# ZhaoyangLyu/Point_Diffusion_Refinement

Measured on AMD Instinct MI355X. Metric: DDPM reverse steps/sec (T=1000, N=2048), higher is better.
Workload: dtype f32; 1 GPU; BASELINE configs[1]: B=32/GPU, N=2048, 3072-pt mirrored condition, T=1000 DDPM reverse sampling, random-init dual-path PointNet++ (9.76 M params), cached condition step; global_batch=32, parallelism=dp1, launch=hipGraph replay, noise=device Philox, execution=fused channel-last HIP

## Files before the change

### point_diffusion_refinement_amd/csrc/fused_layer_ws.hip

```cpp
#include <cstdlib>

#include "layer_tiles.h"

#include <type_traits>

namespace {

typedef float f32x16 __attribute__((ext_vector_type(16)));
typedef float f32x2 __attribute__((ext_vector_type(2)));
typedef float f32x4 __attribute__((ext_vector_type(4)));

#ifdef PDR_LAB_TRACE
__device__ unsigned long long pdr_lab_trace[3][4096];
__device__ unsigned long long pdr_lab_wg[2048][3];
#define PDR_T(role, slot)                                                                   \
  do {                                                                                      \
    if (trace_on && (threadIdx.x & 63) == 0 && (slot) < 4096)                               \
      pdr_lab_trace[role][slot] = __builtin_amdgcn_s_memtime();                             \
  } while (0)
#else
#define PDR_T(role, slot) do {} while (0)
#endif

constexpr int kMaxCin = 4096;
__device__ float k_ones[kMaxCin + 8] = {[0 ... kMaxCin + 7] = 1.0f};
__device__ float k_zeros[kMaxCin + 8] = {[0 ... kMaxCin + 7] = 0.0f};

__device__ __forceinline__ float vmax(float a, float b) {
  float r;
  asm("v_max_f32 %0, %1, %2" : "=v"(r) : "v"(a), "v"(b));
  return r;
}

template <bool SPLIT, int KC, int TM, int TN>
struct StageMem;
template <int KC, int TM, int TN>
struct StageMem<false, KC, TM, TN> {
  static constexpr int APAD = KC == 32 ? 1 : 2;
  __attribute__((aligned(8))) float As[2][KC / 2][TM + APAD][2];
  __attribute__((aligned(16))) float Bs[2][KC][TN];
};
template <int KC, int TM, int TN>
struct StageMem<true, KC, TM, TN> {
  static_assert(KC == 32, "split layout: 32 halves = 64-byte rows");
  __attribute__((aligned(16))) unsigned char A[2][2][TM * 64];
  __attribute__((aligned(16))) unsigned char B[2][2][TN * 64];
};

typedef _Float16 half8 __attribute__((ext_vector_type(8)));
typedef _Float16 half2v __attribute__((ext_vector_type(2)));

__device__ __forceinline__ int split_off(int r, int g) { return r * 64 + ((g ^ ((r >> 2) & 3)) << 4); }

template <int RT, int CT, bool RADD, bool SPLIT>
constexpr int ws_waves_per_simd() { return (RT * CT == 1 && !RADD && !SPLIT) ? 6 : 4; }

template <int RT, int CT, int WR, int WC, int KC, bool RADD, int GATH = 0, bool SPLIT = false, bool POOL = false,
          bool PAIR = false>
__global__ __launch_bounds__(512, (ws_waves_per_simd<RT, CT, RADD, SPLIT>())) void fused_layer_ws_kernel(
    pdr_layer_in_t in_a, int Cin, const float* __restrict__ Wt, int ldw,
    const float* __restrict__ bias, int Cout, float* __restrict__ Y_a, int ldy_a,
    float* __restrict__ partial_a, int relu_col0, int n_row_tiles_a, int tile_order, pdr::PoolArgs pool,
    pdr::WsTwin tw) {
  static_assert(!PAIR || (!RADD && !SPLIT && !POOL && GATH != 2), "paired launches: plain / ball-gathered, no residual");
  const int sel = PAIR ? __builtin_amdgcn_readfirstlane(static_cast<int>(blockIdx.x) >= tw.gx ? 1 : 0) : 0;
  const bool second = PAIR && sel != 0;
  const pdr_layer_in_t& in = PAIR ? tw.in[sel] : in_a;
  float* const __restrict__ Y = PAIR ? tw.Y[sel] : Y_a;
  float* const __restrict__ partial = PAIR ? tw.partial[sel] : partial_a;
  const int ldy = PAIR ? tw.ldy[sel] : ldy_a;
  const int n_row_tiles = PAIR ? tw.n_row_tiles[sel] : n_row_tiles_a;
  const int vbx = (PAIR && second) ? static_cast<int>(blockIdx.x) - tw.gx : static_cast<int>(blockIdx.x);
  const int vnwg = PAIR ? (second ? static_cast<int>(gridDim.x) - tw.gx : tw.gx) : static_cast<int>(gridDim.x);
  static_assert(WR * WC == 4, "4 consumer waves");
  constexpr int TM = WR * RT * 32, TN = WC * CT * 32;
  static_assert(!SPLIT || TN == 128 || TN == 64, "split image: 128- or 64-column blocks");
  constexpr int C4 = KC / 4;
  constexpr int PT = 256;
  constexpr int VSTEP = PT / C4;
  constexpr int APT4 = TM / VSTEP;
  constexpr int TN4 = TN / 4;
  constexpr int WPT4 = (KC * TN4 + PT - 1) / PT;
  static_assert(TM % VSTEP == 0, "tile rows");
  __shared__ StageMem<SPLIT, KC, TM, TN> sm;
  __shared__ float red[WR][TN][2];
  __shared__ int epi_ticket;
  __shared__ __attribute__((aligned(16))) float Tt[4][16][36];

  const int tid = threadIdx.x;
  const int wave = __builtin_amdgcn_readfirstlane(tid >> 6);
  const int rpb = in.rows_per_batch;
  const int tpb = (rpb + TM - 1) / TM;
  const int n0 = blockIdx.y * TN;
  int nch = 0;
  for (int s = 0; s < in.n_seg; ++s) nch += (in.seg[s].C + KC - 1) / KC;
  const int nwg = vnwg;
  const int nB = n_row_tiles / tpb;
  const bool listed = in.tile_list != nullptr;
  const bool xcd_order = !listed && tile_order != 0 && (nwg & 7) == 0 && nB >= 8 && (nB & 7) == 0;
  const int xcd = vbx & 7;
  const int tile_first = xcd_order ? vbx >> 3 : vbx;
  const int tile_step = xcd_order ? nwg >> 3 : nwg;
  const int tile_limit = listed ? min(*in.n_tiles, n_row_tiles)
                                : (xcd_order ? ((nB - xcd + 7) >> 3) * tpb : n_row_tiles);
  const bool rev = in.walk_reverse != 0 && !listed;
  auto row_tile = [&](int l) __attribute__((always_inline)) -> int {
    return listed ? in.tile_list[l] : (rev ? tile_limit - 1 - l : l);
  };
  const int ptpb = in.partial_tpb > 0 ? in.partial_tpb : tpb;
  const int cloud_mul = xcd_order ? 8 : 1, cloud_add = xcd_order ? xcd : 0;
  const int my_tiles = tile_limit > tile_first ? (tile_limit - tile_first + tile_step - 1) / tile_step : 0;
  if constexpr (POOL) {
    if (in.patch_values) {
      constexpr int TN4p = TN / 4;
      constexpr int QP = 512 / TN4p;
      const int Kp = pool.K;
      const long nq = static_cast<long>(n_row_tiles) * TM / Kp;
      const int qpb = rpb / Kp;
      const int c = n0 + 4 * (tid % TN4p);
      const float lo = pool.v_relu ? 0.0f : -__builtin_inff();
      if (tid < QP * TN4p && c < Cout) {
        for (long q = static_cast<long>(blockIdx.x) * QP + tid / TN4p; q < nq; q += static_cast<long>(gridDim.x) * QP) {
          if (in.patch_w[q] > 0.0f) {
            const long bq = q / qpb;
            const f32x4 v = *reinterpret_cast<const f32x4*>(in.patch_values + q * in.patch_ld + c);
            f32x4 sc = {1.0f, 1.0f, 1.0f, 1.0f}, sh = {0.0f, 0.0f, 0.0f, 0.0f};
            if (pool.vscale) sc = *reinterpret_cast<const f32x4*>(pool.vscale + bq * Cout + c);
            if (pool.vshift) sh = *reinterpret_cast<const f32x4*>(pool.vshift + bq * Cout + c);
            f32x4 o;
#pragma unroll
            for (int j = 0; j < 4; ++j) o[j] = vmax(__builtin_fmaf(v[j], sc[j], sh[j]), lo);
            const long orow = in.out_rows ? static_cast<long>(in.out_rows[q]) : q;
            *reinterpret_cast<f32x4*>(pool.out + orow * pool.ldo + c) = o;
          }
        }
      }
    }
  }
  if (my_tiles == 0) return;
#ifdef PDR_LAB_TRACE
  if (tid == 0 && blockIdx.y == 0 && blockIdx.x < 2048) {
    unsigned xcc;
    asm volatile("s_getreg_b32 %0, hwreg(HW_REG_XCC_ID)" : "=s"(xcc));
    pdr_lab_wg[blockIdx.x][0] = __builtin_amdgcn_s_memrealtime();
    pdr_lab_wg[blockIdx.x][2] = (xcc & 15) | (static_cast<unsigned long long>(my_tiles) << 8);
  }
#endif
  const int G = my_tiles * nch;
  const bool has_partial = partial != nullptr;
  if (tid == 0) epi_ticket = 0;
#ifdef PDR_LAB_TRACE
  const bool trace_on = blockIdx.x == 37 % gridDim.x && blockIdx.y == 0 && (wave == 0 || wave == 4 || wave == 6);
#endif

  struct Cur { int tile, sg, ks, cbase, ci; };
  auto advance = [&](Cur& c, bool really = true) {
    const int segC = in.seg[c.sg].C;
    const int ks1 = c.ks + KC;
    const bool seg_end = ks1 >= segC;
    const bool tile_end = seg_end && (c.sg + 1 >= in.n_seg);
    Cur n;
    n.ks = seg_end ? 0 : ks1;
    n.cbase = tile_end ? 0 : (seg_end ? c.cbase + segC : c.cbase);
    n.sg = tile_end ? 0 : (seg_end ? c.sg + 1 : c.sg);
    n.tile = tile_end ? c.tile + tile_step : c.tile;
    n.ci = tile_end ? 0 : c.ci + 1;
    c.ci = really ? n.ci : c.ci;
    c.ks = really ? n.ks : c.ks;
    c.cbase = really ? n.cbase : c.cbase;
    c.sg = really ? n.sg : c.sg;
    c.tile = really ? n.tile : c.tile;
  };
  auto last_of_tile = [&](const Cur& c) { return c.sg == in.n_seg - 1 && c.ks + KC >= in.seg[c.sg].C; };

  if (wave >= 4) {
#ifndef PDR_LAB_NO_PRIO
    __builtin_amdgcn_s_setprio(3);
#endif
    if constexpr (SPLIT) {
      __builtin_amdgcn_s_setreg(1 | (23 << 6) | (0 << 11), 1);
    }
    const float lo_pre = in.pre_relu ? 0.0f : -__builtin_inff();
    const float lo_post = in.post_relu ? 0.0f : -__builtin_inff();
    const int pt = tid - 256;
    const int vc4 = pt % C4, vr0 = pt / C4;
    constexpr bool ROWQ = GATH != 0;
    const int gsh_ = (GATH && in.gK > 0) ? __builtin_ctz(in.gK) : 0;
    auto prow = [&](int i) __attribute__((always_inline)) -> int { return ROWQ ? APT4 * vr0 + i : vr0 + VSTEP * i; };
    const int ss_ld = in.ss_ld > 0 ? in.ss_ld : Cin;
    const bool has_pre = in.pre_relu != 0, has_add = in.add != nullptr;
    unsigned a_off[APT4], r_off[RADD ? APT4 : 1], w_off[WPT4];
    int off_sg = -1;
    {
      const int nmax = ldw - n0 - 4;
#pragma unroll
      for (int i = 0; i < WPT4; ++i) {
        const int e = pt + PT * i;
        const int k = e / TN4, n4 = e - k * TN4;
        w_off[i] = static_cast<unsigned>(min(k, KC - 1) * ldw + min(4 * n4, nmax)) * 4u;
      }
      if constexpr (RADD) {
#pragma unroll
        for (int i = 0; i < APT4; ++i)
          r_off[i] = static_cast<unsigned>(prow(i) * in.rseg.ld + 4 * vc4) * 4u;
      }
    }
    int g_idx[GATH ? APT4 : 1], n_idx[GATH == 1 ? APT4 : 1], n_cnt = 1;
    unsigned v_off = 0;
    auto load_idx = [&](long r0, int nv, int (&id)[GATH ? APT4 : 1], int& cnt) __attribute__((always_inline)) {
      if constexpr (GATH != 0) {
        const int rf = min(APT4 * vr0, nv - 1);
        cnt = in.gcnt ? in.gcnt[(r0 + rf) >> gsh_] : 1;
        if (nv == TM) {
          __builtin_memcpy(&id[0], in.gidx + r0 + APT4 * vr0, sizeof(int) * APT4);
        } else {
#pragma unroll
          for (int i = 0; i < APT4; ++i) id[i] = in.gidx[r0 + min(APT4 * vr0 + i, nv - 1)];
        }
      }
    };
    constexpr bool KNN = GATH == 2;
    float gs1v[KNN ? APT4 : 1], gs2v[KNN ? APT4 : 1];
    f32x4 Rq1, Rq2;
    int g_tile = -1, n_tile = -1;
    const int gsh = (GATH && in.gK > 0) ? __builtin_ctz(in.gK) : 0;
    bool Rgath = false;
    constexpr bool RG = RADD && GATH != 0;
    float4 Rrv[APT4], Rrv2[1];
    f32x4 Rrrv[RADD ? APT4 : 1], Rrrv2[1], Rqr1, Rqr2;
    f32x4 Rrw[WPT4];
    float Rps[4], Rph[4], Rpa[4];
    int Rkmax = KC, Rcvalid = 4;
    auto fetch = [&](const Cur& c) __attribute__((always_inline)) {
      const int lt = row_tile(c.tile);
      const int bl = lt / tpb, tb = lt - bl * tpb;
      const int b = bl * cloud_mul + cloud_add;
#ifdef PDR_LAB_SAME_ROWS
      const long row0 = static_cast<long>(tb & 1) * TM;
#else
      const long row0 = static_cast<long>(b) * rpb + static_cast<long>(tb) * TM;
#endif
      const int nvalid = min(TM, rpb - tb * TM);
      const pdr_seg_t seg = in.seg[c.sg];
      const int shift = __builtin_ctz(seg.row_div);
      Rkmax = min(KC, seg.C - c.ks);
      const float* sc_b = (in.scale ? in.scale + static_cast<long>(b) * ss_ld : k_ones) + c.cbase + c.ks;
      const float* sh_b = (in.shift ? in.shift + static_cast<long>(b) * ss_ld : k_zeros) + c.cbase + c.ks;
      const float* ad_b = (in.add ? in.add + static_cast<long>(b) * in.add_ld : k_zeros) + c.cbase + c.ks;
      const bool f_g = GATH && seg.gV != nullptr;
      if constexpr (GATH) {
        if (c.tile != g_tile && (!PAIR || in.gidx)) {
          off_sg = -1;
          if (GATH == 1 && c.tile == n_tile) {
#pragma unroll
            for (int i = 0; i < APT4; ++i) g_idx[i] = n_cnt <= 0 ? -1 : n_idx[i];
          } else {
            int cnt = 1;
            load_idx(row0, nvalid, g_idx, cnt);
#pragma unroll
            for (int i = 0; i < APT4; ++i) g_idx[i] = cnt <= 0 ? -1 : g_idx[i];
          }
          if constexpr (KNN) {
            if (nvalid == TM) {
              __builtin_memcpy(&gs1v[0], in.gs1 + row0 + APT4 * vr0, sizeof(float) * APT4);
              __builtin_memcpy(&gs2v[0], in.gs2 + row0 + APT4 * vr0, sizeof(float) * APT4);
            } else {
#pragma unroll
              for (int i = 0; i < APT4; ++i) {
                const long p = row0 + min(prow(i), nvalid - 1);
                gs1v[i] = in.gs1[p];
                gs2v[i] = in.gs2[p];
              }
            }
          }
          g_tile = c.tile;
        }
        const int nt = c.tile + tile_step;
        if (GATH == 1 && last_of_tile(c) && nt < tile_limit && (!PAIR || in.gidx)) {
          const int nlt = row_tile(nt);
          const int nbl = nlt / tpb, ntb = nlt - nbl * tpb;
          const int nb = nbl * cloud_mul + cloud_add;
          const long nrow0 = static_cast<long>(nb) * rpb + static_cast<long>(ntb) * TM;
          const int nnv = min(TM, rpb - ntb * TM);
          if constexpr (GATH == 1) load_idx(nrow0, nnv, n_idx, n_cnt);
          n_tile = nt;
        }
      }
      const char* ab = reinterpret_cast<const char*>(
          seg.ptr + (f_g ? static_cast<long>(b) * seg.g_nsrc : (row0 >> shift)) * seg.ld + c.ks);
      const int zrow = f_g ? seg.g_zrow - b * seg.g_nsrc : 0;
      const int v0d = (f_g && seg.gV0) ? static_cast<int>(seg.gV0 - seg.gV) : 0;
      const char* wb = SPLIT ? reinterpret_cast<const char*>(Wt) +
                                   (static_cast<long>(blockIdx.y) * ldw + c.ci) * (2L * TN * 64)
                             : reinterpret_cast<const char*>(Wt + static_cast<long>(c.cbase + c.ks) * ldw + n0);
      unsigned ao[APT4], ro[RADD ? APT4 : 1], wo[WPT4], po[4], vo = 0;
      if (Rkmax == KC && nvalid == TM) {
        if (off_sg != c.sg) {
          off_sg = c.sg;
#pragma unroll
          for (int i = 0; i < APT4; ++i) {
            int row = prow(i) >> shift;
            if constexpr (GATH) {
              if (f_g) {
                row = g_idx[i] < 0 ? zrow : g_idx[i];
                if (i == 0)
                  v_off = static_cast<unsigned>((prow(0) >> gsh) * seg.g_ldv + 4 * vc4 + (g_idx[0] < 0 ? v0d : 0)) * 4u;
              }
            }
            a_off[i] = static_cast<unsigned>(row * seg.ld + 4 * vc4) * 4u;
          }
        }
        if constexpr (GATH) vo = v_off;
        Rcvalid = 4;
#pragma unroll
        for (int j = 0; j < 4; ++j) po[j] = 16u * vc4 + 4u * j;
#pragma unroll
        for (int i = 0; i < APT4; ++i) ao[i] = a_off[i];
        if constexpr (RADD) {
#pragma unroll
          for (int i = 0; i < APT4; ++i) ro[i] = r_off[i];
        }
#pragma unroll
        for (int i = 0; i < WPT4; ++i) wo[i] = SPLIT ? static_cast<unsigned>(pt + PT * i) * 16u : w_off[i];
      } else {
        const int cl = 4 * vc4;
        const int clc = min(cl, ((seg.C + 3) & ~3) - 4 - c.ks);
        Rcvalid = cl == clc ? min(4, seg.C - c.ks - clc) : 0;
#pragma unroll
        for (int j = 0; j < 4; ++j) po[j] = static_cast<unsigned>(min(clc + j, seg.C - 1 - c.ks)) * 4u;
#pragma unroll
        for (int i = 0; i < APT4; ++i) {
          const int r = min(prow(i), nvalid - 1);
          int row = r >> shift;
          if constexpr (GATH) {
            if (f_g) {
              row = g_idx[i] < 0 ? zrow : g_idx[i];
              if (i == 0) vo = static_cast<unsigned>((r >> gsh) * seg.g_ldv + clc + (g_idx[0] < 0 ? v0d : 0)) * 4u;
            }
          }
          ao[i] = static_cast<unsigned>(row * seg.ld + clc) * 4u;
          if constexpr (RADD) ro[i] = static_cast<unsigned>(r * in.rseg.ld + clc) * 4u;
        }
        const int nmax = ldw - n0 - 4;
#pragma unroll
        for (int i = 0; i < WPT4; ++i) {
          const int e = pt + PT * i;
          const int k = e / TN4, n4 = e - k * TN4;
          wo[i] = SPLIT ? static_cast<unsigned>(pt + PT * i) * 16u
                        : static_cast<unsigned>(min(k, Rkmax - 1) * ldw + min(4 * n4, nmax)) * 4u;
        }
      }
      if (Rkmax == KC) {
        f32x4 s4, h4, a4;
        __builtin_memcpy(&s4, reinterpret_cast<const char*>(sc_b) + 16u * vc4, 16);
        __builtin_memcpy(&h4, reinterpret_cast<const char*>(sh_b) + 16u * vc4, 16);
        __builtin_memcpy(&a4, reinterpret_cast<const char*>(ad_b) + 16u * vc4, 16);
#pragma unroll
        for (int j = 0; j < 4; ++j) {
          Rps[j] = s4[j];
          Rph[j] = h4[j];
          Rpa[j] = a4[j];
        }
      } else {
#pragma unroll
        for (int j = 0; j < 4; ++j) {
          Rps[j] = *reinterpret_cast<const float*>(reinterpret_cast<const char*>(sc_b) + po[j]);
          Rph[j] = *reinterpret_cast<const float*>(reinterpret_cast<const char*>(sh_b) + po[j]);
          Rpa[j] = *reinterpret_cast<const float*>(reinterpret_cast<const char*>(ad_b) + po[j]);
        }
      }
#pragma unroll
      for (int i = 0; i < APT4; ++i) Rrv[i] = *reinterpret_cast<const float4*>(ab + ao[i]);
      if constexpr (GATH) {
        Rgath = f_g;
        if (f_g) {
          const char* vb = reinterpret_cast<const char*>(seg.gV + (row0 >> gsh) * seg.g_ldv + c.ks);
          Rrv2[0] = *reinterpret_cast<const float4*>(vb + vo);
          if constexpr (KNN) {
            const unsigned qo = Rkmax == KC ? 16u * vc4
                                            : static_cast<unsigned>(min(4 * vc4, ((seg.C + 3) & ~3) - 4 - c.ks)) * 4u;
            __builtin_memcpy(&Rq1, reinterpret_cast<const char*>(seg.g_r1 + c.ks) + qo, 16);
            __builtin_memcpy(&Rq2, reinterpret_cast<const char*>(seg.g_r2 + c.ks) + qo, 16);
          }
        }
      }
      if constexpr (RG) {
        const int rs_ld = in.rseg.ld, rs_ldv = in.rseg.g_ldv, rs_nsrc = in.rseg.g_nsrc;
        const char* rb = reinterpret_cast<const char*>(in.rseg.ptr + static_cast<long>(b) * rs_nsrc * rs_ld +
                                                       c.cbase + c.ks);
        const char* rvb = reinterpret_cast<const char*>(in.rseg.gV + (row0 >> gsh) * rs_ldv + c.cbase + c.ks);
        const int rz = in.rseg.g_zrow - b * rs_nsrc;
        const int rv0d = in.rseg.gV0 ? static_cast<int>(in.rseg.gV0 - in.rseg.gV) : 0;
        const bool fast = Rkmax == KC && nvalid == TM;
        const int colq = fast ? 4 * vc4 : min(4 * vc4, ((Cin + 3) & ~3) - 4 - c.cbase - c.ks);
#pragma unroll
        for (int i = 0; i < APT4; ++i) {
          const int urow = g_idx[i] < 0 ? rz : g_idx[i];
          Rrrv[i] = *reinterpret_cast<const f32x4*>(rb + static_cast<unsigned>(urow * rs_ld + colq) * 4u);
        }
        Rrrv2[0] = *reinterpret_cast<const f32x4*>(
            rvb + static_cast<unsigned>((min(prow(0), nvalid - 1) >> gsh) * rs_ldv + colq +
                                        (g_idx[0] < 0 ? rv0d : 0)) * 4u);
        if constexpr (GATH == 2) {
          __builtin_memcpy(&Rqr1, in.rseg.g_r1 + c.cbase + c.ks + colq, 16);
          __builtin_memcpy(&Rqr2, in.rseg.g_r2 + c.cbase + c.ks + colq, 16);
        }
      } else if constexpr (RADD) {
        const char* rb = reinterpret_cast<const char*>(in.rseg.ptr + row0 * in.rseg.ld + c.cbase + c.ks);
#pragma unroll
        for (int i = 0; i < APT4; ++i) Rrrv[i] = *reinterpret_cast<const f32x4*>(rb + ro[i]);
      }
#pragma unroll
      for (int i = 0; i < WPT4; ++i) Rrw[i] = *reinterpret_cast<const f32x4*>(wb + wo[i]);
    };
    auto commit = [&](int st) __attribute__((always_inline)) {
      auto stage_a = [&](auto masked, auto pre, auto add) __attribute__((always_inline)) {
        constexpr bool MASKED = decltype(masked)::value, PRE = decltype(pre)::value, ADD = decltype(add)::value;
#pragma unroll
        for (int i = 0; i < APT4; ++i) {
          float x[4] = {Rrv[i].x, Rrv[i].y, Rrv[i].z, Rrv[i].w};
          if constexpr (GATH) {
            if (Rgath) {
              x[0] += Rrv2[0].x; x[1] += Rrv2[0].y; x[2] += Rrv2[0].z; x[3] += Rrv2[0].w;
              if constexpr (KNN) {
#pragma unroll
                for (int j = 0; j < 4; ++j) {
                  x[j] = __builtin_fmaf(gs1v[i], Rq1[j], x[j]);
                  x[j] = __builtin_fmaf(gs2v[i], Rq2[j], x[j]);
                }
              }
            }
          }
          float q[4] = {0.0f, 0.0f, 0.0f, 0.0f};
          if constexpr (RADD) {
            q[0] = Rrrv[i][0]; q[1] = Rrrv[i][1]; q[2] = Rrrv[i][2]; q[3] = Rrrv[i][3];
            if constexpr (RG) {
              q[0] += Rrrv2[0][0]; q[1] += Rrrv2[0][1]; q[2] += Rrrv2[0][2]; q[3] += Rrrv2[0][3];
              if constexpr (GATH == 2) {
#pragma unroll
                for (int j = 0; j < 4; ++j) {
                  q[j] = __builtin_fmaf(gs1v[i], Rqr1[j], q[j]);
                  q[j] = __builtin_fmaf(gs2v[i], Rqr2[j], q[j]);
                }
              }
            }
          }
#pragma unroll
          for (int j = 0; j < 4; ++j) {
            float v = x[j];
            if constexpr (PRE) v = vmax(v, lo_pre);
            v = __builtin_fmaf(v, Rps[j], Rph[j]);
            v = vmax(v, lo_post);
            if constexpr (ADD) v = v + Rpa[j];
            if constexpr (RADD) v = v + q[j];
            if constexpr (MASKED) v = j < Rcvalid ? v : 0.0f;
            x[j] = v;
          }
          if constexpr (!SPLIT) {
            *reinterpret_cast<f32x2*>(&sm.As[st][2 * vc4][prow(i)][0]) = f32x2{x[0], x[1]};
            *reinterpret_cast<f32x2*>(&sm.As[st][2 * vc4 + 1][prow(i)][0]) = f32x2{x[2], x[3]};
          }
          if constexpr (SPLIT) {
            typedef float f2 __attribute__((ext_vector_type(2)));
            const f2 v01 = {x[0], x[1]}, v23 = {x[2], x[3]};
            const half2v h01 = __builtin_convertvector(v01, half2v), h23 = __builtin_convertvector(v23, half2v);
            const f2 r01 = v01 - __builtin_convertvector(h01, f2), r23 = v23 - __builtin_convertvector(h23, f2);
            const half2v l01 = __builtin_convertvector(r01, half2v), l23 = __builtin_convertvector(r23, half2v);
            const int r = prow(i);
            const int off = split_off(r, vc4 >> 1) + ((vc4 & 1) << 3);
            typedef unsigned u2 __attribute__((ext_vector_type(2)));
            *reinterpret_cast<u2*>(&sm.A[st][0][off]) =
                u2{__builtin_bit_cast(unsigned, h01), __builtin_bit_cast(unsigned, h23)};
            *reinterpret_cast<u2*>(&sm.A[st][1][off]) =
                u2{__builtin_bit_cast(unsigned, l01), __builtin_bit_cast(unsigned, l23)};
          }
        }
      };
      using T = std::true_type;
      using F = std::false_type;
      if (Rkmax < KC) stage_a(T(), T(), T());
      else if (has_pre) stage_a(F(), T(), T());
      else if (has_add) stage_a(F(), F(), T());
      else stage_a(F(), F(), F());
      if constexpr (SPLIT) {
        unsigned char* wdst = &sm.B[st][0][0];
#pragma unroll
        for (int i = 0; i < WPT4; ++i) *reinterpret_cast<f32x4*>(wdst + (pt + PT * i) * 16) = Rrw[i];
      } else {
#pragma unroll
        for (int i = 0; i < WPT4; ++i) {
          const int e = pt + PT * i;
          const int k = e / TN4, n4 = e - k * TN4;
          if (KC * TN4 % PT == 0 || e < KC * TN4) *reinterpret_cast<f32x4*>(&sm.Bs[st][k][4 * n4]) = Rrw[i];
        }
      }
    };

    Cur co{tile_first, 0, 0, 0, 0};
    fetch(co);
    for (int g = 0; g < G; ++g) {
      PDR_T(1, 4 * g + 0);
#ifdef PDR_LAB_TRACE
      asm volatile("s_waitcnt vmcnt(0)" ::: "memory");
      PDR_T(1, 4 * g + 3);
#endif
      commit(g & 1);
      PDR_T(1, 4 * g + 1);
      advance(co, g + 1 < G);
      fetch(co);
      PDR_T(1, 4 * g + 2);
      __syncthreads();
    }
    return;
  }

  const int lane = tid & 63;
  const int wr = wave % WR, wc = wave / WR;
  const int il = lane & 31, hi = lane >> 5;
  float bias_r[CT];
#pragma unroll
  for (int j = 0; j < CT; ++j) {
    const int col = n0 + (wc * CT + j) * 32 + il;
    bias_r[j] = (bias && col < Cout) ? bias[col] : 0.0f;
  }
  f32x16 acc[RT][CT];
#pragma unroll
  for (int i = 0; i < RT; ++i)
#pragma unroll
    for (int j = 0; j < CT; ++j)
#pragma unroll
      for (int r = 0; r < 16; ++r) acc[i][j][r] = bias_r[j];

  Cur cur{tile_first, 0, 0, 0, 0};
  for (int g = 0; g < G; ++g) {
    PDR_T(0, 4 * g + 0);
    __syncthreads();
    PDR_T(0, 4 * g + 1);
    const int st = g & 1;
    if constexpr (SPLIT) {
      const int ksteps16 = (min(KC, in.seg[cur.sg].C - cur.ks) + 15) >> 4;
      for (int ks = 0; ks < ksteps16; ++ks) {
        half8 ah[RT], al[RT], wh[CT], wl[CT];
        const int gq = 2 * ks + hi;
#pragma unroll
        for (int i = 0; i < RT; ++i) {
          const int off = split_off((wr * RT + i) * 32 + il, gq);
          ah[i] = *reinterpret_cast<const half8*>(&sm.A[st][0][off]);
          al[i] = *reinterpret_cast<const half8*>(&sm.A[st][1][off]);
        }
#pragma unroll
        for (int j = 0; j < CT; ++j) {
          const int off = split_off((wc * CT + j) * 32 + il, gq);
          wh[j] = *reinterpret_cast<const half8*>(&sm.B[st][0][off]);
          wl[j] = *reinterpret_cast<const half8*>(&sm.B[st][1][off]);
        }
#pragma unroll
        for (int i = 0; i < RT; ++i)
#pragma unroll
          for (int j = 0; j < CT; ++j) {
            acc[i][j] = __builtin_amdgcn_mfma_f32_32x32x16_f16(al[i], wh[j], acc[i][j], 0, 0, 0);
            acc[i][j] = __builtin_amdgcn_mfma_f32_32x32x16_f16(ah[i], wl[j], acc[i][j], 0, 0, 0);
            acc[i][j] = __builtin_amdgcn_mfma_f32_32x32x16_f16(ah[i], wh[j], acc[i][j], 0, 0, 0);
          }
      }
    } else {
      const int kquads = (min(KC, in.seg[cur.sg].C - cur.ks) + 3) >> 2;
      for (int kq = 0; kq < kquads; ++kq) {
        f32x2 a[RT];
        float w0[CT], w1[CT];
#pragma unroll
        for (int i = 0; i < RT; ++i)
          a[i] = *reinterpret_cast<const f32x2*>(&sm.As[st][2 * kq + hi][(wr * RT + i) * 32 + il][0]);
#pragma unroll
        for (int j = 0; j < CT; ++j) {
          w0[j] = sm.Bs[st][4 * kq + 2 * hi][(wc * CT + j) * 32 + il];
          w1[j] = sm.Bs[st][4 * kq + 2 * hi + 1][(wc * CT + j) * 32 + il];
        }
#pragma unroll
        for (int i = 0; i < RT; ++i)
#pragma unroll
          for (int j = 0; j < CT; ++j) {
            acc[i][j] = __builtin_amdgcn_mfma_f32_32x32x2f32(a[i].x, w0[j], acc[i][j], 0, 0, 0);
            acc[i][j] = __builtin_amdgcn_mfma_f32_32x32x2f32(a[i].y, w1[j], acc[i][j], 0, 0, 0);
          }
      }
    }
    PDR_T(0, 4 * g + 2);
    if (last_of_tile(cur)) {
      const int lt = row_tile(cur.tile);
      const int bl = lt / tpb, tb = lt - bl * tpb;
      const int b = bl * cloud_mul + cloud_add;
      const int tile = b * ptpb + tb;
#ifdef PDR_LAB_SAME_OUT
      const long row0 = static_cast<long>(blockIdx.x & 511) * TM;
#else
      const long row0 = static_cast<long>(b) * rpb + static_cast<long>(tb) * TM;
#endif
      const int nvalid = min(TM, rpb - tb * TM);
      constexpr bool WSTAT = GATH == 0 || PAIR;
      const int osh = in.oadd ? __builtin_ctz(in.oadd_div) : 0;
      const bool rows_full = nvalid == TM && !(WSTAT && (in.wrow0 || (in.oadd_rows && osh < 5)));
      int il_e = il, hi_e = hi, lane_e = lane;
      asm volatile("" : "+v"(il_e), "+v"(hi_e), "+v"(lane_e));
      long ldy_e = ldy;
      asm volatile("" : "+s"(ldy_e));
      if constexpr (POOL) {
        const int K = pool.K, ksh = __builtin_ctz(K);
        const float lo = pool.v_relu ? 0.0f : -__builtin_inff();
        const long vrow_bytes = static_cast<long>(pool.ldv) * 4;
#pragma unroll
        for (int i = 0; i < RT; ++i) {
          const long rb = row0 + (wr * RT + i) * 32;
          int cn[4];
#pragma unroll
          for (int g4 = 0; g4 < 4; ++g4) {
            int c = K;
            if (pool.counts) {
              c = pool.counts[(rb + 8 * g4) >> ksh];
              c = c < 1 ? 1 : c;
            }
            cn[g4] = c;
          }
#pragma unroll
          for (int j = 0; j < CT; ++j) {
            const int col = n0 + (wc * CT + j) * 32 + il_e;
            const bool colok = col < Cout;
            const int cc = colok ? col : 0;
            float v[16];
            {
              unsigned voff = static_cast<unsigned>(4 * hi_e * pool.ldv + cc) * 4u;
              asm volatile("" : "+v"(voff));
              const char* q = reinterpret_cast<const char*>(pool.values + rb * pool.ldv);
#pragma unroll
              for (int r = 0; r < 16; ++r) {
                if (r > 0) q += ((r & 3) == 0 ? 5 : 1) * vrow_bytes;
                v[r] = *reinterpret_cast<const float*>(q + voff);
              }
            }
            const float vs = pool.vscale ? pool.vscale[static_cast<long>(b) * Cout + cc] : 1.0f;
            const float vh = pool.vshift ? pool.vshift[static_cast<long>(b) * Cout + cc] : 0.0f;
#pragma unroll
            for (int r = 0; r < 16; ++r) {
              const int kk = ((r & 3) + 8 * (r >> 2) + 4 * hi_e) & (K - 1);
              acc[i][j][r] = (kk < cn[r >> 2] ? acc[i][j][r] : -1e9f) * 1.44269504088896340736f;
              v[r] = vmax(__builtin_fmaf(v[r], vs, vh), lo);
            }
            auto reduce = [&](auto gsz_c) __attribute__((always_inline)) {
              constexpr int GSZ = decltype(gsz_c)::value;
#pragma unroll
              for (int g = 0; g < 4; g += GSZ) {
                float m = -__builtin_inff();
#pragma unroll
                for (int r = 4 * g; r < 4 * (g + GSZ); ++r) m = fmaxf(m, acc[i][j][r]);
                m = fmaxf(m, __shfl_xor(m, 32, 64));
                float l = 0.0f, a = 0.0f;
#pragma unroll
                for (int r = 4 * g; r < 4 * (g + GSZ); ++r) {
                  const float w = __builtin_amdgcn_exp2f(acc[i][j][r] - m);
                  l += w;
                  a = __builtin_fmaf(v[r], w, a);
                }
                l += __shfl_xor(l, 32, 64);
                a += __shfl_xor(a, 32, 64);
                if (hi_e == 0 && colok) {
                  const long q = (rb + 8 * g) >> ksh;
                  pool.out[(in.out_rows ? static_cast<long>(in.out_rows[q]) : q) * pool.ldo + col] = a / l;
                }
              }
            };
            if (K == 8) reduce(std::integral_constant<int, 1>());
            else if (K == 16) reduce(std::integral_constant<int, 2>());
            else reduce(std::integral_constant<int, 4>());
            float bj = bias_r[j];
            asm volatile("" : "+v"(bj));
#pragma unroll
            for (int r = 0; r < 16; ++r) acc[i][j][r] = bj;
            __builtin_amdgcn_sched_barrier(0);
          }
        }
      } else {
#pragma unroll
      for (int j = 0; j < CT; ++j) {
        const int cl = (wc * CT + j) * 32 + il_e;
        const int col = n0 + cl;
        const bool colok = col < Cout;
        const int c0 = n0 + (wc * CT + j) * 32;
        float s1 = 0.0f, s2 = 0.0f;
        if (rows_full) {
          if (in.oadd) {
            const float* ob = in.oadd + (colok ? col : 0);
            if (osh >= 5) {
#pragma unroll
              for (int i = 0; i < RT; ++i) {
                long oq = (row0 + (wr * RT + i) * 32) >> osh;
                if constexpr (GATH != 2) oq = in.oadd_rows ? static_cast<long>(in.oadd_rows[oq]) : oq;
                const float v = ob[oq * in.oadd_ld];
#pragma unroll
                for (int r = 0; r < 16; ++r) acc[i][j][r] += v;
              }
            } else {
#pragma unroll
              for (int i = 0; i < RT; ++i)
#pragma unroll
                for (int r = 0; r < 16; ++r) {
                  const int rl = (wr * RT + i) * 32 + (r & 3) + 8 * (r >> 2) + 4 * hi_e;
                  acc[i][j][r] += ob[((row0 + rl) >> osh) * in.oadd_ld];
                }
            }
          }
          const unsigned lane_off = static_cast<unsigned>(4 * hi_e * ldy + col) * 4u;
          const long row_bytes = ldy_e * 4;
          const bool none_relu = c0 + 32 <= relu_col0, all_relu = c0 >= relu_col0;
          const bool wide_store = (ldy & 3) == 0 && (reinterpret_cast<uintptr_t>(Y) & 15) == 0;
          const int rr = lane_e >> 3, c4 = (lane_e & 7) * 4;
          const bool col4ok = c0 + c4 < ((Cout + 3) & ~3);
          unsigned toff = static_cast<unsigned>(rr * ldy + c0 + c4) * 4u;
          asm volatile("" : "+v"(toff));
          auto store_tile = [&](auto mode, auto wide) {
            constexpr int MODE = decltype(mode)::value;
            constexpr bool WIDE = decltype(wide)::value;
            const float lo = (MODE == 2 && col < relu_col0) ? -__builtin_inff() : 0.0f;
#pragma unroll
            for (int i = 0; i < RT; ++i) {
              char* q = reinterpret_cast<char*>(Y + (row0 + (wr * RT + i) * 32) * ldy_e);
#pragma unroll
              for (int h = 0; h < 2; ++h) {
#pragma unroll
                for (int r8 = 0; r8 < 8; ++r8) {
                  const float y = acc[i][j][8 * h + r8];
                  if (WIDE) {
                    Tt[wave][8 * (r8 >> 2) + (r8 & 3) + 4 * hi_e][il_e] = y;
                  } else {
                    if (h + r8 > 0) q += ((r8 & 3) == 0 ? 5 : 1) * row_bytes;
                    if (colok) *reinterpret_cast<float*>(q + lane_off) = y;
                  }
                }
                if (colok) {
#pragma unroll
                  for (int r8 = 0; r8 < 8; ++r8) {
                    const float y = acc[i][j][8 * h + r8];
                    const float f = MODE == 0 ? y : vmax(y, lo);
                    s1 += f;
                    s2 = __builtin_fmaf(f, f, s2);
                  }
                }
                if (WIDE) {
                  const f32x4 v0 = *reinterpret_cast<const f32x4*>(&Tt[wave][rr][c4]);
                  const f32x4 v1 = *reinterpret_cast<const f32x4*>(&Tt[wave][rr + 8][c4]);
                  if (col4ok) {
                    char* qh = q + (16 * h) * row_bytes;
#if defined(PDR_LAB_NT_STORE)
                    __builtin_nontemporal_store(v0, reinterpret_cast<f32x4*>(qh + toff));
                    __builtin_nontemporal_store(v1, reinterpret_cast<f32x4*>(qh + 8 * row_bytes + toff));
#elif !defined(PDR_LAB_NO_STORE)
                    *reinterpret_cast<f32x4*>(qh + toff) = v0;
                    *reinterpret_cast<f32x4*>(qh + 8 * row_bytes + toff) = v1;
#endif
                  }
                }
              }
            }
          };
          using M0 = std::integral_constant<int, 0>;
          using M1 = std::integral_constant<int, 1>;
          using M2 = std::integral_constant<int, 2>;
#ifdef PDR_LAB_DIRECT_STORE
          if (RT * CT == 4) {
            if (none_relu) store_tile(M0(), std::false_type());
            else if (all_relu) store_tile(M1(), std::false_type());
            else store_tile(M2(), std::false_type());
          } else
#endif
          if (wide_store) {
            if (none_relu) store_tile(M0(), std::true_type());
            else if (all_relu) store_tile(M1(), std::true_type());
            else store_tile(M2(), std::true_type());
          } else {
            store_tile(M2(), std::false_type());
          }
        } else {
          int wlo = 0;
          if constexpr (WSTAT) wlo = in.wrow0 ? in.wrow0[b] - tb * TM : 0;
          const bool relu_stat = col >= relu_col0;
          float* ybase = Y + row0 * ldy + col;
          const float* ob = in.oadd ? in.oadd + (colok ? col : 0) : nullptr;
          if (colok) {
#pragma unroll
            for (int i = 0; i < RT; ++i) {
#pragma unroll
              for (int r = 0; r < 16; ++r) {
                const int rl = (wr * RT + i) * 32 + (r & 3) + 8 * (r >> 2) + 4 * hi_e;
                if (rl < nvalid) {
                  float y = acc[i][j][r];
                  if (ob) {
                    long oq = (row0 + rl) >> osh;
                    if constexpr (WSTAT) oq = in.oadd_rows ? static_cast<long>(in.oadd_rows[oq]) : oq;
                    y += ob[oq * in.oadd_ld];
                  }
                  ybase[rl * ldy] = y;
                  if (rl >= wlo) {
                    const float f = relu_stat ? fmaxf(y, 0.0f) : y;
                    s1 += f;
                    s2 = __builtin_fmaf(f, f, s2);
                  }
                }
                __builtin_amdgcn_sched_barrier(0);
              }
            }
          }
          if constexpr (WSTAT) {
            if (in.wrow0) {
              s1 *= in.wmul;
              s2 *= in.wmul;
            }
          }
        }
        PDR_T(2, 8 * (g / nch) + j);
        if (has_partial) {
          s1 += __shfl_xor(s1, 32, 64);
          s2 += __shfl_xor(s2, 32, 64);
          if (hi_e == 0) {
            red[wr][cl][0] = s1;
            red[wr][cl][1] = s2;
          }
        }
        float bj = bias_r[j];
        asm volatile("" : "+v"(bj));
#pragma unroll
        for (int i = 0; i < RT; ++i)
#pragma unroll
          for (int r = 0; r < 16; ++r) acc[i][j][r] = bj;
      }
      }
      PDR_T(2, 8 * (g / nch) + 6);
      if (has_partial) {
        int ticket = 0;
        if (lane == 0)
          ticket = __hip_atomic_fetch_add(&epi_ticket, 1, __ATOMIC_ACQ_REL, __HIP_MEMORY_SCOPE_WORKGROUP);
        ticket = __builtin_amdgcn_readfirstlane(ticket);
        if ((ticket & 3) == 3) {
          for (int c = lane; c < TN; c += 64) {
            if (n0 + c < Cout) {
              float s1 = 0.0f, s2 = 0.0f;
#pragma unroll
              for (int w = 0; w < WR; ++w) {
                s1 += red[w][c][0];
                s2 += red[w][c][1];
              }
              float* o = partial + (static_cast<long>(tile) * Cout + n0 + c) * 2;
              o[0] = s1;
              o[1] = s2;
            }
          }
        }
      }
    }
    PDR_T(0, 4 * g + 3);
    advance(cur);
  }
#ifdef PDR_LAB_TRACE
  if (tid == 0 && blockIdx.y == 0 && blockIdx.x < 2048) pdr_lab_wg[blockIdx.x][1] = __builtin_amdgcn_s_memrealtime();
#endif
}

}

#ifdef PDR_LAB_TRACE
extern "C" int pdr_lab_wg_read(unsigned long long* dst) {
  return hipMemcpyFromSymbol(dst, HIP_SYMBOL(pdr_lab_wg), sizeof(unsigned long long) * 2048 * 3) == hipSuccess ? 0 : -1;
}
extern "C" int pdr_lab_trace_read(unsigned long long* dst) {
  return hipMemcpyFromSymbol(dst, HIP_SYMBOL(pdr_lab_trace), sizeof(unsigned long long) * 3 * 4096) == hipSuccess ? 0 : -1;
}
#endif

namespace pdr {

bool fused_layer_ws_supported(int id, const LayerSource& src, const pdr_layer_in_t& in, int Cin) {
  const bool radd = src.radd, gath = src.gath, knn = src.knn, knn_res = src.knn_res;
  if (Cin > kMaxCin) return false;
  if (in.wrow0 && gath) return false;
  if (id < 0 || id >= kNumTiles) return false;
  const int tm_map = tile_tm(id) > 128 ? tile_tm(id) : 128;
  if (in.oadd_rows && gath && (in.oadd_div < 32 || in.rows_per_batch % tm_map != 0)) return false;
  if (!tile_has_ws(id)) return false;
  if (in.oadd_rows && (knn || knn_res)) return false;
  if (knn) {
    if (!gath || radd || !in.gs1 || !in.gs2 || in.gcnt) return false;
    for (int sg = 0; sg < in.n_seg; ++sg)
      if (in.seg[sg].gV && (!in.seg[sg].g_r1 || !in.seg[sg].g_r2)) return false;
  }
  if (knn_res && (!in.gs1 || !in.gs2 || in.gcnt || !in.rseg.g_r2)) return false;
  if (gath) {
    if (in.gK < 4) return false;
    bool main_g = false;
    for (int sg = 0; sg < in.n_seg; ++sg) main_g = main_g || in.seg[sg].gV != nullptr;
    if (radd && main_g) return false;
    if (in.rseg.gV && (main_g || knn || !in.gidx)) return false;
    for (int sg = 0; sg <= in.n_seg; ++sg) {
      const pdr_seg_t& g = sg < in.n_seg ? in.seg[sg] : in.rseg;
      if (!g.gV) continue;
      if (in.gcnt) {
        if (g.g_zrow < 0 || !g.gV0) return false;
        const long d = g.gV0 - g.gV;
        if (d < 0 || d >= (1L << 28)) return false;
      }
    }
  }
  return true;
}

}

namespace {

struct WsArgs {
  dim3 grid; hipStream_t s; const pdr_layer_in_t& in; int Cin; const float* Wt; int ldw; const float* bias; int Cout;
  float* Y; int ldy; float* partial; int relu_col0, n_row_tiles, tile_order; pdr::PoolArgs pool; pdr::WsTwin twin;
};

template <class T, bool RADD, int GATH, bool SPLIT, bool POOL = false, bool PAIR = false>
void ws_launch(const WsArgs& a) {
  hipLaunchKernelGGL((fused_layer_ws_kernel<T::RT, T::CT, T::WR, T::WC, T::KC, RADD, GATH, SPLIT, POOL, PAIR>), a.grid,
                     dim3(512), 0, a.s, a.in, a.Cin, a.Wt, a.ldw, a.bias, a.Cout, a.Y, a.ldy, a.partial, a.relu_col0,
                     a.n_row_tiles, a.tile_order, a.pool, a.twin);
}

template <class T, bool SPLIT>
void ws_launch_form(const WsArgs& a, const pdr::LayerSource& src) {
  if (src.gath && src.knn) ws_launch<T, false, 2, SPLIT>(a);
  else if (src.gath && src.radd && src.knn_res) ws_launch<T, true, 2, SPLIT>(a);
  else if (src.gath && src.radd) ws_launch<T, true, 1, SPLIT>(a);
  else if (src.gath) ws_launch<T, false, 1, SPLIT>(a);
  else if (src.radd) ws_launch<T, true, 0, SPLIT>(a);
  else ws_launch<T, false, 0, SPLIT>(a);
}

}

namespace pdr {

void launch_fused_layer_ws(int id, const LayerSource& src, const pdr_layer_in_t& in, int Cin, const float* Wt, int ldw,
                           const float* bias, int Cout, float* Y, int ldy, float* partial, int relu_col0,
                           int n_row_tiles, int ncol, hipStream_t s, bool split, const PoolArgs* pool) {
  long gx = n_row_tiles;
  const bool narrow3 = pdr::option(pdr::OPT_WS_NARROW3) != 0;
  const long resident = (narrow3 && id == 7 && !src.radd && !split) ? 768 : 512;
  const int xcd_knob = pdr::option(pdr::OPT_WS_XCD_ORDER);
  const int tile_order = (xcd_knob >= 2 || (xcd_knob == 1 && src.gath)) ? 1 : 0;
  long cap = (resident + ncol - 1) / ncol;
  int tile_order_eff = tile_order;
  if (tile_order && cap >= 8) cap = cap / 8 * 8;
  else tile_order_eff = 0;
  if (gx > cap) gx = cap;
  if (gx < 1) gx = 1;
  const WsArgs a{dim3(static_cast<unsigned>(gx), static_cast<unsigned>(ncol)), s, in, Cin, Wt, ldw, bias, Cout, Y, ldy,
                 partial, relu_col0, n_row_tiles, tile_order_eff, pool ? *pool : PoolArgs(), WsTwin()};
  with_tile(id, [&](auto t) {
    using T = decltype(t);
    if constexpr (tile_has_ws(T::id)) {
      if constexpr (tile_has_split(T::id)) {
        if (split) {
          if (pool) ws_launch<T, false, 0, true, true>(a);
          else ws_launch_form<T, true>(a, src);
          return;
        }
      }
      if (pool) ws_launch<T, false, 0, false, true>(a);
      else ws_launch_form<T, false>(a, src);
    }
  });
}

void launch_fused_layer_ws_pair(int id, bool gath, const pdr_layer_in_t& in, int Cin, const float* Wt, int ldw,
                                const float* bias, int Cout, float* Y, int ldy, float* partial, int relu_col0,
                                int n_row_tiles, int ncol, WsTwin twin, hipStream_t s) {
  const long resident = 512;
  long cap = (resident + ncol - 1) / ncol;
  long gx1 = n_row_tiles < cap ? n_row_tiles : cap;
  long gx2 = twin.n_row_tiles[1] < cap ? twin.n_row_tiles[1] : cap;
  if (gx1 < 1) gx1 = 1;
  if (gx2 < 1) gx2 = 1;
  twin.gx = static_cast<int>(gx1);
  twin.in[0] = in;
  twin.Y[0] = Y;
  twin.partial[0] = partial;
  twin.ldy[0] = ldy;
  twin.n_row_tiles[0] = n_row_tiles;
  const WsArgs a{dim3(static_cast<unsigned>(gx1 + gx2), static_cast<unsigned>(ncol)), s, in, Cin, Wt, ldw, bias, Cout,
                 Y, ldy, partial, relu_col0, n_row_tiles, 0, PoolArgs(), twin};
  with_tile(id, [&](auto t) {
    using T = decltype(t);
    if constexpr (tile_has_pair(T::id)) {
      if (gath) ws_launch<T, false, 1, false, false, true>(a);
      else ws_launch<T, false, 0, false, false, true>(a);
    }
  });
}

}
```

Before: 6062 cloud-steps/s.

## Stream weight tiles into LDS via global_load_lds DMA in producer waves

Producer waves now load the weight tile straight from global memory into LDS with global_load_lds instead of reading it into registers and writing it out to LDS during commit. The weight DMA for the next stage is issued after the barrier. A hand-counted s_waitcnt vmcnt leaves the activation loads outstanding while the DMA for the current stage must complete. The aim is to free the producers' weight registers and their LDS store instructions and to overlap the weight fetch. The risk is that the hardcoded vmcnt counts are wrong for some template variant, which would race on LDS.

```diff
diff --git a/point_diffusion_refinement_amd/csrc/fused_layer_ws.hip b/point_diffusion_refinement_amd/csrc/fused_layer_ws.hip
--- a/point_diffusion_refinement_amd/csrc/fused_layer_ws.hip
+++ b/point_diffusion_refinement_amd/csrc/fused_layer_ws.hip
@@ -20,6 +20,12 @@
   } while (0)
 #else
 #define PDR_T(role, slot) do {} while (0)
+#endif
+
+#ifdef PDR_LAB_W_REGS
+constexpr bool kWDma = false;
+#else
+constexpr bool kWDma = true;
 #endif
 
 constexpr int kMaxCin = 4096;
@@ -228,9 +234,41 @@
     constexpr bool RG = RADD && GATH != 0;
     float4 Rrv[APT4], Rrv2[1];
     f32x4 Rrrv[RADD ? APT4 : 1], Rrrv2[1], Rqr1, Rqr2;
-    f32x4 Rrw[WPT4];
+    f32x4 Rrw[kWDma ? 1 : WPT4];
     float Rps[4], Rph[4], Rpa[4];
     int Rkmax = KC, Rcvalid = 4;
+    auto w_source = [&](const Cur& c, int kmax, unsigned (&wo)[WPT4]) __attribute__((always_inline)) -> const char* {
+      if (SPLIT || kmax == KC) {
+#pragma unroll
+        for (int i = 0; i < WPT4; ++i) wo[i] = SPLIT ? static_cast<unsigned>(pt + PT * i) * 16u : w_off[i];
+      } else {
+        const int nmax = ldw - n0 - 4;
+#pragma unroll
+        for (int i = 0; i < WPT4; ++i) {
+          const int e = pt + PT * i;
+          const int k = e / TN4, n4 = e - k * TN4;
+          wo[i] = static_cast<unsigned>(min(k, kmax - 1) * ldw + min(4 * n4, nmax)) * 4u;
+        }
+      }
+      return SPLIT ? reinterpret_cast<const char*>(Wt) + (static_cast<long>(blockIdx.y) * ldw + c.ci) * (2L * TN * 64)
+                   : reinterpret_cast<const char*>(Wt + static_cast<long>(c.cbase + c.ks) * ldw + n0);
+    };
+    static_assert((KC * TN4) % 64 == 0, "W image: whole 64-lane DMA pieces");
+    auto dma_w = [&](const Cur& c, int st) __attribute__((always_inline)) {
+      unsigned wo[WPT4];
+      const char* wb = w_source(c, min(KC, in.seg[c.sg].C - c.ks), wo);
+      typedef __attribute__((address_space(3))) unsigned char lds_byte;
+      lds_byte* img;
+      if constexpr (SPLIT) img = (lds_byte*)&sm.B[st][0][0];
+      else img = (lds_byte*)&sm.Bs[st][0][0];
+#pragma unroll
+      for (int i = 0; i < WPT4; ++i) {
+        const int e0 = 64 * (wave - 4) + PT * i;
+        if (KC * TN4 % PT == 0 || e0 < KC * TN4)
+          __builtin_amdgcn_global_load_lds((const __attribute__((address_space(1))) void*)(wb + wo[i]), img + 16 * e0, 16,
+                                           0, 0);
+      }
+    };
     auto fetch = [&](const Cur& c) __attribute__((always_inline)) {
       const int lt = row_tile(c.tile);
       const int bl = lt / tpb, tb = lt - bl * tpb;
@@ -290,10 +328,7 @@
           seg.ptr + (f_g ? static_cast<long>(b) * seg.g_nsrc : (row0 >> shift)) * seg.ld + c.ks);
       const int zrow = f_g ? seg.g_zrow - b * seg.g_nsrc : 0;
       const int v0d = (f_g && seg.gV0) ? static_cast<int>(seg.gV0 - seg.gV) : 0;
-      const char* wb = SPLIT ? reinterpret_cast<const char*>(Wt) +
-                                   (static_cast<long>(blockIdx.y) * ldw + c.ci) * (2L * TN * 64)
-                             : reinterpret_cast<const char*>(Wt + static_cast<long>(c.cbase + c.ks) * ldw + n0);
-      unsigned ao[APT4], ro[RADD ? APT4 : 1], wo[WPT4], po[4], vo = 0;
+      unsigned ao[APT4], ro[RADD ? APT4 : 1], po[4], vo = 0;
       if (Rkmax == KC && nvalid == TM) {
         if (off_sg != c.sg) {
           off_sg = c.sg;
@@ -320,8 +355,6 @@
 #pragma unroll
           for (int i = 0; i < APT4; ++i) ro[i] = r_off[i];
         }
-#pragma unroll
-        for (int i = 0; i < WPT4; ++i) wo[i] = SPLIT ? static_cast<unsigned>(pt + PT * i) * 16u : w_off[i];
       } else {
         const int cl = 4 * vc4;
         const int clc = min(cl, ((seg.C + 3) & ~3) - 4 - c.ks);
@@ -340,14 +373,6 @@
           }
           ao[i] = static_cast<unsigned>(row * seg.ld + clc) * 4u;
           if constexpr (RADD) ro[i] = static_cast<unsigned>(r * in.rseg.ld + clc) * 4u;
-        }
-        const int nmax = ldw - n0 - 4;
-#pragma unroll
-        for (int i = 0; i < WPT4; ++i) {
-          const int e = pt + PT * i;
-          const int k = e / TN4, n4 = e - k * TN4;
-          wo[i] = SPLIT ? static_cast<unsigned>(pt + PT * i) * 16u
-                        : static_cast<unsigned>(min(k, Rkmax - 1) * ldw + min(4 * n4, nmax)) * 4u;
         }
       }
       if (Rkmax == KC) {
@@ -410,8 +435,12 @@
 #pragma unroll
         for (int i = 0; i < APT4; ++i) Rrrv[i] = *reinterpret_cast<const f32x4*>(rb + ro[i]);
       }
-#pragma unroll
-      for (int i = 0; i < WPT4; ++i) Rrw[i] = *reinterpret_cast<const f32x4*>(wb + wo[i]);
+      if constexpr (!kWDma) {
+        unsigned wo[WPT4];
+        const char* wb = w_source(c, Rkmax, wo);
+#pragma unroll
+        for (int i = 0; i < WPT4; ++i) Rrw[i] = *reinterpret_cast<const f32x4*>(wb + wo[i]);
+      }
     };
     auto commit = [&](int st) __attribute__((always_inline)) {
       auto stage_a = [&](auto masked, auto pre, auto add) __attribute__((always_inline)) {
@@ -482,7 +511,8 @@
       else if (has_pre) stage_a(F(), T(), T());
       else if (has_add) stage_a(F(), F(), T());
       else stage_a(F(), F(), F());
-      if constexpr (SPLIT) {
+      if constexpr (kWDma) {
+      } else if constexpr (SPLIT) {
         unsigned char* wdst = &sm.B[st][0][0];
 #pragma unroll
         for (int i = 0; i < WPT4; ++i) *reinterpret_cast<f32x4*>(wdst + (pt + PT * i) * 16) = Rrw[i];
@@ -496,9 +526,12 @@
       }
     };
 
+    constexpr int NVM = 3 + APT4 + (RADD ? APT4 : 0) + (RG ? 1 + (GATH == 2 ? 2 : 0) : 0);
+    constexpr int NVM_G = NVM + 1 + (KNN ? 2 : 0);
     Cur co{tile_first, 0, 0, 0, 0};
     fetch(co);
-    for (int g = 0; g < G; ++g) {
+    if constexpr (kWDma) dma_w(co, 0);
+    for (int g = 0;; ++g) {
       PDR_T(1, 4 * g + 0);
 #ifdef PDR_LAB_TRACE
       asm volatile("s_waitcnt vmcnt(0)" ::: "memory");
@@ -509,7 +542,16 @@
       advance(co, g + 1 < G);
       fetch(co);
       PDR_T(1, 4 * g + 2);
-      __syncthreads();
+      if constexpr (kWDma) {
+        if (GATH != 0 && Rgath) asm volatile("s_waitcnt vmcnt(%0) lgkmcnt(0)" ::"n"(NVM_G) : "memory");
+        else asm volatile("s_waitcnt vmcnt(%0) lgkmcnt(0)" ::"n"(NVM) : "memory");
+        __builtin_amdgcn_s_barrier();
+        if (g + 1 >= G) break;
+        dma_w(co, (g + 1) & 1);
+      } else {
+        __syncthreads();
+        if (g + 1 >= G) break;
+      }
     }
     return;
   }
```

After: 6177 cloud-steps/s (median of 6 runs). +1.9%, better.
